# morgana-proofs/GKR-MSM

Measured on AMD Instinct MI355X. Metric: msm_points_per_sec, higher is better.
Workload: dtype u32 limbs, u64 column accumulators (BLS12-381 Fr in Montgomery form: 9 x 29-bit limbs in registers, 8 x 32 in memory)

## Files before the change

### gkr_msm_amd/csrc/g1.hip

```cpp
#include <string.h>

#include <cstring>
#include <mutex>
#include <thread>
#include <vector>


#include "common.hpp"
#include "internal.hpp"
#include "g1.hip.h"
#include "sort.hip.h"
#include "msm_plan.hpp"

namespace gm {

static constexpr uint32_t G1_NEG_BIT = 0x80000000u;

__global__ void __launch_bounds__(256) k_g1_lower_bound(const uint32_t* __restrict__ keys, uint64_t ntasks, uint32_t nkeys,
                                                         uint32_t* __restrict__ off, uint32_t* __restrict__ max_len) {
    const uint32_t k = blockIdx.x * blockDim.x + threadIdx.x;
    if (k > nkeys) return;
    auto lb = [&](uint32_t key) {
        uint64_t lo = 0, hi = ntasks;
        while (lo < hi) {
// ... 386 lines not shown

__global__ void __launch_bounds__(256) k_g1_map_tasks(const uint32_t* __restrict__ mapping, uint64_t n, uint32_t nkeys,
                                                       uint32_t* __restrict__ keys, uint32_t* __restrict__ idx,
                                                       uint32_t* __restrict__ bad) {
    const uint64_t i = (uint64_t)blockIdx.x * blockDim.x + threadIdx.x;
    if (i >= n) return;
    const uint32_t m = mapping[i];
    if (m >= nkeys) atomicAdd(bad, 1u);
    keys[i] = m < nkeys ? m : nkeys;
    idx[i] = (uint32_t)i;
}

__global__ void __launch_bounds__(128) k_g1_to_affine(const G1Jac* __restrict__ in, uint64_t n, G1Aff* __restrict__ out) {
    const uint64_t i = (uint64_t)blockIdx.x * blockDim.x + threadIdx.x;
    if (i >= n) return;
    g1_aff_store(out + i, g1_to_aff(g1_load(in + i)));
}

__global__ void __launch_bounds__(128) k_g1_from_affine(const G1Aff* __restrict__ in, uint64_t n, G1Jac* __restrict__ out) {
    const uint64_t i = (uint64_t)blockIdx.x * blockDim.x + threadIdx.x;
    if (i >= n) return;
    g1_store(out + i, g1_from_aff(g1_aff_load(in + i)));
}

__global__ void __launch_bounds__(128) k_g1_gen_points(G1Aff gen, uint64_t n, uint64_t seed, G1Aff* __restrict__ out) {
    const uint64_t i = (uint64_t)blockIdx.x * blockDim.x + threadIdx.x;
    if (i >= n) return;
    uint64_t z = seed + 0x9E3779B97F4A7C15ULL * (i + 1);
    z = (z ^ (z >> 30)) * 0xBF58476D1CE4E5B9ULL;
    z = (z ^ (z >> 27)) * 0x94D049BB133111EBULL;
    z ^= z >> 31;
    z |= 1;
    G1Jac acc = g1_inf();
    for (int b = 63; b >= 0; b--) {
        acc = g1_dbl(acc);
        if ((z >> b) & 1) acc = g1_add_mixed(acc, gen);
    }
    g1_aff_store(out + i, g1_to_aff(acc));
}

__global__ void __launch_bounds__(128) k_g1_mock_srs(G1Aff g0, Fr tau, uint64_t n, G1Aff* __restrict__ out) {
    const uint64_t i = (uint64_t)blockIdx.x * blockDim.x + threadIdx.x;
    if (i >= n) return;
    Fr acc = fr_one(), b = tau;
    for (uint64_t e = i; e; e >>= 1) {
        if (e & 1) acc = fr_mul(acc, b);
        b = fr_sqr(b);
    }
    const Fr k = fr_from_mont(acc);
    G1Jac r = g1_inf();
    for (int li = 7; li >= 0; li--)
        for (int bit = 31; bit >= 0; bit--) {
            r = g1_dbl(r);
            if ((k.l[li] >> bit) & 1) r = g1_add_mixed(r, g0);
        }
    g1_aff_store(out + i, g1_to_aff(r));
}

struct G1Scratch {
    char* base = nullptr;
    size_t cap = 0, used = 0;
    std::mutex mu;
    int32_t reserve(size_t bytes) {
        if (bytes <= cap) return GM_OK;
        if (base) dev_free(base);
        base = nullptr;
        cap = 0;
        hipError_t e = dev_alloc((void**)&base, bytes);
        if (e != hipSuccess) return set_err(GM_ERR_HIP, "hipMalloc(G1 scratch %zu): %s", bytes, hipGetErrorString(e));
        cap = bytes;
        return GM_OK;
    }
    void* carve(size_t b) {
        const size_t a = (used + 255) & ~(size_t)255;
        used = a + b;
        return base + a;
    }
    void release() {
        if (base) dev_free(base);
        base = nullptr;
        cap = used = 0;
    }
};
static G1Scratch& g1_scratch() {
    static G1Scratch s[GM_MAX_DEVICES];
    int dev = 0;
    (void)hipGetDevice(&dev);
    return s[(dev >= 0 && dev < GM_MAX_DEVICES) ? dev : 0];
}

static size_t al(size_t b) { return (b + 255) & ~(size_t)255; }

struct G1Layout {
    size_t sort_tmp = 0, scan_tmp = 0, total = 0;
};

static uint32_t bit_len(uint32_t v) {
    uint32_t b = 0;
    while (v) { b++; v >>= 1; }
    return b;
}

static int32_t g1_engine_layout(uint64_t ntasks, uint32_t nkeys, G1Layout* L) {
    const size_t st = radix_sort_tmp_bytes(ntasks), sc = 33 * scan_tmp_bytes((size_t)nkeys + 1);
    L->sort_tmp = st;
    L->scan_tmp = sc;
    L->total = al(st) + al(sc) + 2 * al(ntasks * 4) + 35 * al(((size_t)nkeys + 1) * 4) + al(64) + al((ntasks / 64 + (size_t)34 * (nkeys / 32 + 3) + 64) * 4) +
               al((ntasks / 2 + nkeys + 1) * (size_t)G1_CELL_WORDS * 4) + al((ntasks / 4 + nkeys + 1) * (size_t)G1_CELL_WORDS * 4) + 4096;
    return GM_OK;
}

static int32_t g1_sum_by_key(G1Scratch& ws, const G1Aff* src_aff, const G1Jac* src_jac, uint32_t* keys, uint32_t* idx,
                             uint64_t ntasks, uint32_t nkeys, G1Jac* out, hipStream_t s) {
    GM_REQUIRE(ntasks < (1ull << 31), "too many G1 tasks (%llu)", (unsigned long long)ntasks);
    GM_REQUIRE(nkeys >= 1 && nkeys < (1u << 30), "bad key count %u", nkeys);
    G1Layout L;
    int32_t rc = g1_engine_layout(ntasks ? ntasks : 1, nkeys, &L);
    if (rc) return rc;
    uint32_t* sort_tmp = (uint32_t*)ws.carve(L.sort_tmp);
    uint32_t* scan_tmp = (uint32_t*)ws.carve(L.scan_tmp);
    uint32_t* keys_s = (uint32_t*)ws.carve((ntasks + 1) * 4);
    uint32_t* idx_s = (uint32_t*)ws.carve((ntasks + 1) * 4);
    const size_t orow = (size_t)nkeys + 1;
    uint32_t* off_all = (uint32_t*)ws.carve(33 * al(orow * 4));
    const size_t ostride = al(orow * 4) / 4;
    (void)ws.carve(orow * 4);
    uint32_t* d_max = (uint32_t*)ws.carve(64);
    uint32_t* bufA = (uint32_t*)ws.carve((ntasks / 2 + nkeys + 1) * (size_t)G1_CELL_WORDS * 4);
    uint32_t* bufB = (uint32_t*)ws.carve((ntasks / 4 + nkeys + 1) * (size_t)G1_CELL_WORDS * 4);
    uint32_t* blk_row = (uint32_t*)ws.carve((ntasks / 64 + (size_t)34 * (nkeys / 32 + 3) + 64) * 4);
    if (ws.used > ws.cap) return set_err(GM_ERR_STATE, "G1 scratch under-reserved (%zu > %zu)", ws.used, ws.cap);

    GM_HIP(hipMemsetAsync(d_max, 0, 4, s));
    GM_HIP(radix_sort_pairs_u32(keys, idx, keys_s, idx_s, ntasks, bit_len(nkeys), sort_tmp, &keys_s, &idx_s, s));
    hipLaunchKernelGGL(k_g1_lower_bound, dim3(ceil_div(orow, 256)), dim3(256), 0, s, keys_s, ntasks, nkeys, off_all, d_max);
    GM_LAUNCH_CHECK();
    uint32_t max_len = 0;
    GM_HIP(hipMemcpyAsync(&max_len, d_max, 4, hipMemcpyDeviceToHost, s));
    GM_HIP(hipStreamSynchronize(s));
    uint32_t nlev = 0;
    while ((1u << nlev) < max_len) nlev++;
    GM_REQUIRE(nlev <= 32, "row too long");
    if (nlev) {
        const uint32_t ntiles = ceil_div(orow, SCAN_TILE);
        hipLaunchKernelGGL(k_g1_levels_scan_tiles, dim3(ntiles, nlev), dim3(1024), 0, s, off_all, nkeys, off_all, ostride, scan_tmp);
        GM_LAUNCH_CHECK();
        if (ntiles > 1) {
            hipLaunchKernelGGL(k_g1_levels_scan_fix, dim3(ntiles, nlev), dim3(1024), 0, s, nkeys, off_all, ostride, scan_tmp);
            GM_LAUNCH_CHECK();
        }
    }
    const G1SrcAff sa{src_aff, idx_s};
    const G1SrcJac sj{src_jac, idx_s};
    if (nlev == 0) {
        if (src_aff) hipLaunchKernelGGL((k_g1_rows_out<G1SrcAff>), dim3(ceil_div(nkeys, 128)), dim3(128), 0, s, sa, off_all, nkeys, out);
        else hipLaunchKernelGGL((k_g1_rows_out<G1SrcJac>), dim3(ceil_div(nkeys, 128)), dim3(128), 0, s, sj, off_all, nkeys, out);
        GM_LAUNCH_CHECK();
        return GM_OK;
    }
    uint64_t bound = ntasks / 2 + nkeys;
    G1BlockRowsArgs ba;
    ba.nlev = nlev;
    {
        uint64_t b = bound;
        uint32_t tot = 0;
        for (uint32_t l = 0; l < nlev; l++) {
            ba.first[l] = tot;
// ... 174 lines not shown
struct G1FixedBase {
    const G1Aff* bases = nullptr;
    uint64_t n = 0;
    uint32_t c = 16, nwin = 16;
    G1Aff* tab = nullptr;
    int dev = 0;
    G1Aff first{}, last{};
};
static std::mutex& g1_fixed_mu() {
    static std::mutex m;
    return m;
}
static std::vector<G1FixedBase>& g1_fixed_registry() {
    static std::vector<G1FixedBase> r;
    return r;
}
static bool g1_fixed_lookup(const G1Aff* bases, uint64_t n, G1FixedBase* out, hipStream_t s) {
    G1FixedBase cand;
    {
        std::lock_guard<std::mutex> lock(g1_fixed_mu());
        bool found = false;
        int dev = 0;
        (void)hipGetDevice(&dev);
        for (const G1FixedBase& f : g1_fixed_registry())
            if (f.bases == bases && n <= f.n && f.dev == dev) { cand = f; found = true; break; }
        if (!found) return false;
    }
    G1Aff now[2];
    if (hipMemcpyAsync(&now[0], cand.bases, sizeof(G1Aff), hipMemcpyDeviceToHost, s) != hipSuccess ||
        hipMemcpyAsync(&now[1], cand.bases + (cand.n - 1), sizeof(G1Aff), hipMemcpyDeviceToHost, s) != hipSuccess ||
        hipStreamSynchronize(s) != hipSuccess) {
        (void)hipGetLastError();
        return false;
    }
    if (memcmp(&now[0], &cand.first, sizeof(G1Aff)) != 0 || memcmp(&now[1], &cand.last, sizeof(G1Aff)) != 0) return false;
    *out = cand;
    return true;
}

static int32_t g1_msm_fixed_core(const G1FixedBase& fb, const uint64_t* d_scalars, uint64_t n, int scalars_mont, uint32_t nbits,
                                 G1Jac* h_out, hipStream_t s) {
    if (n == 0) { *h_out = g1_inf(); return GM_OK; }
    GM_REQUIRE(nbits >= 1 && nbits <= 256, "bad scalar width %u", nbits);
    uint32_t nwin = (nbits + fb.c - 1) / fb.c;
    if (nwin > fb.nwin) nwin = fb.nwin;
    const uint64_t ntasks = (uint64_t)nwin * n;
    const uint32_t nkeys = 1u << fb.c;
    GM_REQUIRE(ntasks < (1ull << 31) && fb.n * fb.nwin < (1ull << 31), "fixed-base MSM too large for one call");
    G1Scratch& ws = g1_scratch();
    std::lock_guard<std::mutex> lock(ws.mu);
    const size_t need = 2 * al(ntasks * 4) + al((size_t)nkeys * sizeof(G1Jac)) + g1_engine_bytes(ntasks, nkeys) +
                        g1_weighted_bytes(1, nkeys) + 8192;
    int32_t rc = ws.reserve(need);
    if (rc) return rc;
    ws.used = 0;
    uint32_t* keys = (uint32_t*)ws.carve(ntasks * 4);
    uint32_t* idx = (uint32_t*)ws.carve(ntasks * 4);
    G1Jac* buckets = (G1Jac*)ws.carve((size_t)nkeys * sizeof(G1Jac));
    hipLaunchKernelGGL(k_g1_msm_tasks_fixed, dim3(ceil_div(n, 256)), dim3(256), 0, s, reinterpret_cast<const uint32_t*>(d_scalars), n,
                       fb.n, fb.c, nwin, scalars_mont, nkeys, keys, idx);
    GM_LAUNCH_CHECK();
    const size_t mark = ws.used;
    rc = g1_sum_by_key(ws, fb.tab, nullptr, keys, idx, ntasks, nkeys, buckets, s);
    if (rc) return rc;
    ws.used = mark;
    std::vector<G1Jac> wsum;
    rc = g1_weighted_sums(ws, buckets, 1, nkeys, &wsum, s);
    if (rc) return rc;
    *h_out = wsum[0];
    return GM_OK;
}

}

using namespace gm;

static void put_aff(uint64_t* h, const G1Jac& p) {
    const G1Aff a = g1_to_aff(p);
    memcpy(h, &a, sizeof(G1Aff));
}

extern "C" int32_t gm_g1_release_scratch(void) {
    G1Scratch& ws = g1_scratch();
    std::lock_guard<std::mutex> lock(ws.mu);
    ws.release();
    return GM_OK;
}

extern "C" int32_t gm_g1_host(int32_t op, const uint64_t* h_a, const uint64_t* h_b, uint64_t* h_out, uint64_t n) {
    GM_REQUIRE(op >= 0 && op <= 7 && h_a && h_out, "bad argument");
    GM_REQUIRE(!(op == 0 || op == 2 || op == 4 || op == 6 || op == 7) || h_b, "second operand missing");
    for (uint64_t i = 0; i < n; i++) {
        G1Jac ja, jb, jr;
        G1Aff aa, ab, ar;
        switch (op) {
            case 0: memcpy(&ja, h_a + 18 * i, 144); memcpy(&jb, h_b + 18 * i, 144); jr = g1_add(ja, jb); memcpy(h_out + 18 * i, &jr, 144); break;
            case 1: memcpy(&ja, h_a + 18 * i, 144); jr = g1_dbl(ja); memcpy(h_out + 18 * i, &jr, 144); break;
            case 2: memcpy(&ja, h_a + 18 * i, 144); memcpy(&ab, h_b + 12 * i, 96); jr = g1_add_mixed(ja, ab); memcpy(h_out + 18 * i, &jr, 144); break;
            case 3: memcpy(&ja, h_a + 18 * i, 144); ar = g1_to_aff(ja); memcpy(h_out + 12 * i, &ar, 96); break;
            case 4: memcpy(&aa, h_a + 12 * i, 96); memcpy(&ab, h_b + 12 * i, 96); jr = g1_add_aff(aa, ab); memcpy(h_out + 18 * i, &jr, 144); break;
            case 5: memcpy(&aa, h_a + 12 * i, 96); h_out[i] = g1_aff_on_curve(aa) ? 1 : 0; break;
            default: {
                Fq x, y;
                memcpy(&x, h_a + 6 * i, 48); memcpy(&y, h_b + 6 * i, 48);
                const Fq z = op == 6 ? fq_mul(x, y) : fq_mul_c(x, y);
                memcpy(h_out + 6 * i, &z, 48);
            }
        }
    }
    return GM_OK;
}

namespace gm {
__global__ void __launch_bounds__(128) k_g1_batch(int op, const uint64_t* __restrict__ a, const uint64_t* __restrict__ b,
                                                   uint64_t* __restrict__ out, uint64_t n) {
    const uint64_t i = (uint64_t)blockIdx.x * blockDim.x + threadIdx.x;
    if (i >= n) return;
    const G1Jac* ja = reinterpret_cast<const G1Jac*>(a);
    const G1Jac* jb = reinterpret_cast<const G1Jac*>(b);
    const G1Aff* aa = reinterpret_cast<const G1Aff*>(a);
    const G1Aff* ab = reinterpret_cast<const G1Aff*>(b);
    G1Jac* jo = reinterpret_cast<G1Jac*>(out);
    switch (op) {
        case 0: g1_store(jo + i, g1_add(g1_load(ja + i), g1_load(jb + i))); break;
        case 1: g1_store(jo + i, g1_dbl(g1_load(ja + i))); break;
        case 2: g1_store(jo + i, g1_add_mixed(g1_load(ja + i), g1_aff_load(ab + i))); break;
        case 3: g1_aff_store(reinterpret_cast<G1Aff*>(out) + i, g1_to_aff(g1_load(ja + i))); break;
        default: g1_store(jo + i, g1_add_aff(g1_aff_load(aa + i), g1_aff_load(ab + i))); break;
    }
}
}

extern "C" int32_t gm_g1_batch(int32_t op, const uint64_t* d_a, const uint64_t* d_b, uint64_t* d_out, uint64_t n, void* stream) {
    GM_REQUIRE(op >= 0 && op <= 4 && d_a && d_out, "bad argument");
    GM_REQUIRE(!(op == 0 || op == 2 || op == 4) || d_b, "second operand missing");
    if (n == 0) return GM_OK;
    hipLaunchKernelGGL(k_g1_batch, dim3(ceil_div(n, 128)), dim3(128), 0, as_stream(stream), op, d_a, d_b, d_out, n);
    GM_LAUNCH_CHECK();
    return GM_OK;
}

extern "C" int32_t gm_g1_gen_points(uint64_t* d_points_aff, uint64_t n, uint64_t seed, void* stream) {
    GM_REQUIRE(d_points_aff, "null argument");
    if (n == 0) return GM_OK;
    static const uint32_t GX[12] = {0xdb22c6bbu, 0xfb3af00au, 0xf97a1aefu, 0x6c55e83fu, 0x171bac58u, 0xa14e3a3fu,
                                    0x9774b905u, 0xc3688c4fu, 0x4fa9ac0fu, 0x2695638cu, 0x3197d794u, 0x17f1d3a7u};
    static const uint32_t GY[12] = {0x46c5e7e1u, 0x0caa2329u, 0xa2888ae4u, 0xd03cc744u, 0x2c04b3edu, 0x00db18cbu,
                                    0xd5d00af6u, 0xfcf5e095u, 0x741d8ae4u, 0xa09e30edu, 0xe3aaa0f1u, 0x08b3f481u};
    G1Aff g;
    memcpy(&g.x, GX, 48);
    memcpy(&g.y, GY, 48);
    g.x = fq_to_mont(g.x);
    g.y = fq_to_mont(g.y);
    GM_REQUIRE(g1_aff_on_curve(g), "generator constant is off the curve");
    hipLaunchKernelGGL(k_g1_gen_points, dim3(ceil_div(n, 128)), dim3(128), 0, as_stream(stream), g, n, seed,
                       reinterpret_cast<G1Aff*>(d_points_aff));
    GM_LAUNCH_CHECK();
    return GM_OK;
}

extern "C" int32_t gm_g1_generator(uint64_t* h_out_aff) {
    GM_REQUIRE(h_out_aff, "null argument");
    static const uint32_t X[12] = {0xdb22c6bbu, 0xfb3af00au, 0xf97a1aefu, 0x6c55e83fu, 0x171bac58u, 0xa14e3a3fu,
                                   0x9774b905u, 0xc3688c4fu, 0x4fa9ac0fu, 0x2695638cu, 0x3197d794u, 0x17f1d3a7u};
    static const uint32_t Y[12] = {0x46c5e7e1u, 0x0caa2329u, 0xa2888ae4u, 0xd03cc744u, 0x2c04b3edu, 0x00db18cbu,
                                   0xd5d00af6u, 0xfcf5e095u, 0x741d8ae4u, 0xa09e30edu, 0xe3aaa0f1u, 0x08b3f481u};
    G1Aff g;
    for (int i = 0; i < 12; i++) { g.x.l[i] = X[i]; g.y.l[i] = Y[i]; }
// ... 413 lines not shown
```

### gkr_msm_amd/csrc/msm.hip

```cpp
#include <algorithm>
#include <vector>

#include "algfn.hip.h"
#include "common.hpp"
#include "msm_plan.hpp"
#include "ragged.hip.h"
#include "fr9.hip.h"

namespace gm {

static constexpr int CHUNK = 1024;

struct Point3 {
    Fr x, y, z;
};
typedef uint32_t gm_u4_t __attribute__((ext_vector_type(4)));

__device__ __forceinline__ Point3 pt_identity() {
    Point3 p;
    p.x = fr_zero();
    p.y = fr_one();
    p.z = fr_one();
    return p;
}
// ... 1022 lines not shown
#undef STAGE_MARK
    return GM_OK;
}

extern "C" int32_t gm_msm_bucket_sums(const gm_msm_plan* p, const uint64_t** d_x, const uint64_t** d_y,
                                      const uint64_t** d_z, uint64_t* n_rows_local) {
    GM_REQUIRE(p, "null plan");
    if (d_x) *d_x = reinterpret_cast<const uint64_t*>(p->bsum[0]);
    if (d_y) *d_y = reinterpret_cast<const uint64_t*>(p->bsum[1]);
    if (d_z) *d_z = reinterpret_cast<const uint64_t*>(p->bsum[2]);
    if (n_rows_local) *n_rows_local = p->nrows;
    return GM_OK;
}

extern "C" int32_t gm_msm_window_points(const gm_msm_plan* p, const uint64_t** d_cols, uint64_t* n_cols,
                                        uint64_t* col_len) {
    GM_REQUIRE(p, "null plan");
    if (d_cols) *d_cols = reinterpret_cast<const uint64_t*>(p->win_pts);
    if (n_cols) *n_cols = 3ull * (p->d_log + 1);
    if (col_len) *col_len = p->nwin;
    return GM_OK;
}

extern "C" int32_t gm_msm_digits(const gm_msm_plan* p, const uint16_t** d_digits, const uint32_t** d_counter,
                                 const uint32_t** d_row_len) {
    GM_REQUIRE(p, "null plan");
    if (d_digits) *d_digits = p->digits;
    if (d_counter) *d_counter = p->counter;
    if (d_row_len) *d_row_len = p->row_len;
    return GM_OK;
}

namespace gm {

__global__ void __launch_bounds__(256) k_u_to_fr(const uint16_t* __restrict__ dg, const uint32_t* __restrict__ ct,
                                                  uint64_t n, Fr* __restrict__ d_out, Fr* __restrict__ c_out) {
    const uint64_t i = (uint64_t)blockIdx.x * blockDim.x + threadIdx.x;
    if (i >= n) return;
    fr_store(d_out + i, fr_from_u64(dg[i]));
    fr_store(c_out + i, fr_from_u64(ct[i]));
}

__global__ void __launch_bounds__(256) k_access_counts(const uint16_t* __restrict__ dg, const uint32_t* __restrict__ ct,
                                                        uint64_t n, uint32_t* __restrict__ cnt_d, uint32_t* __restrict__ cnt_c) {
    const uint64_t i = (uint64_t)blockIdx.x * blockDim.x + threadIdx.x;
    if (i >= n) return;
    atomicAdd(&cnt_d[dg[i]], 1u);
    atomicAdd(&cnt_c[ct[i]], 1u);
}

__global__ void __launch_bounds__(256) k_neg_count_to_fr(const uint32_t* __restrict__ cnt, uint64_t n, Fr* __restrict__ out) {
    const uint64_t i = (uint64_t)blockIdx.x * blockDim.x + threadIdx.x;
    if (i >= n) return;
    fr_store(out + i, fr_neg(fr_from_u64(cnt[i])));
}

__global__ void __launch_bounds__(256) k_ac_c_from_sorted(const uint32_t* __restrict__ sorted, uint32_t n, uint64_t N, Fr* __restrict__ out) {
    const uint64_t k = (uint64_t)blockIdx.x * blockDim.x + threadIdx.x;
    if (k >= N) return;
    uint32_t lo = 0, hi = n;
    while (lo < hi) {
        const uint32_t mid = (lo + hi) >> 1;
        if (sorted[mid] <= k) lo = mid + 1; else hi = mid;
    }
    fr_store(out + k, fr_neg(fr_from_u64(n - lo)));
}

__global__ void __launch_bounds__(256) k_pull(const uint16_t* __restrict__ dg, const uint32_t* __restrict__ ct, uint64_t n,
                                               const Fr* __restrict__ eq_d, const Fr* __restrict__ eq_c,
                                               Fr* __restrict__ d_pull, Fr* __restrict__ c_pull) {
    const uint64_t i = (uint64_t)blockIdx.x * blockDim.x + threadIdx.x;
    if (i >= n) return;
    fr_store(d_pull + i, fr_load(eq_d + dg[i]));
    fr_store(c_pull + i, fr_load(eq_c + ct[i]));
}

int32_t launch_eq_sequence(const Fr& mult, const Fr* pt, uint32_t nvars, Fr* const* levels, hipStream_t s, const Fr* extra = nullptr,
                           uint32_t n_extra = 0, Fr* extra_dst = nullptr);

}

extern "C" int32_t gm_msm_phase1_polys(const gm_msm_plan* p, uint64_t* d_c, uint64_t* d_d, uint64_t* d_ac_c,
                                       uint64_t* d_ac_d, void* stream) {
    GM_REQUIRE(p && d_c && d_d && d_ac_c && d_ac_d, "null argument");
    hipStream_t s = as_stream(stream);
    const uint64_t n = (uint64_t)p->nwin * p->N;
    hipLaunchKernelGGL(k_u_to_fr, dim3(ceil_div(n, 256)), dim3(256), 0, s, p->digits, p->counter, n,
                       reinterpret_cast<Fr*>(d_d), reinterpret_cast<Fr*>(d_c));
    GM_LAUNCH_CHECK();
    uint32_t* cnt = nullptr;
    const uint64_t nc = (uint64_t)p->nrows + p->nd;
    GM_HIP(dev_alloc((void**)&cnt, nc * 4));
    {
        std::vector<uint32_t> rl(p->nrows), h(nc, 0);
        GM_HIP(hipMemcpyAsync(rl.data(), p->row_len, (size_t)p->nrows * 4, hipMemcpyDeviceToHost, s));
        GM_HIP(hipStreamSynchronize(s));
        for (uint32_t r = 0; r < p->nrows; r++) h[p->nrows + (r % p->nd)] += rl[r];
        std::sort(rl.begin(), rl.end());
        memcpy(h.data(), rl.data(), (size_t)p->nrows * 4);
        GM_HIP(hipMemcpyAsync(cnt, h.data(), nc * 4, hipMemcpyHostToDevice, s));
        GM_HIP(hipStreamSynchronize(s));
    }
    hipLaunchKernelGGL(k_ac_c_from_sorted, dim3(ceil_div(p->N, 256)), dim3(256), 0, s, cnt, p->nrows, p->N, reinterpret_cast<Fr*>(d_ac_c));
    GM_LAUNCH_CHECK();
    hipLaunchKernelGGL(k_neg_count_to_fr, dim3(ceil_div(p->nd, 256)), dim3(256), 0, s, cnt + p->nrows, (uint64_t)p->nd,
                       reinterpret_cast<Fr*>(d_ac_d));
    GM_LAUNCH_CHECK();
    GM_HIP(hipStreamSynchronize(s));
    dev_free(cnt);
    return GM_OK;
}

extern "C" int32_t gm_msm_second_phase(const gm_msm_plan* p, const uint64_t* h_r, uint32_t y_logsize, uint64_t* d_c_pull,
                                       uint64_t* d_d_pull, void* stream) {
    GM_REQUIRE(p && h_r && d_c_pull && d_d_pull, "null argument");
    hipStream_t s = as_stream(stream);
    const uint32_t dl = p->d_log, xl = p->x_log;
    std::vector<Fr> r(y_logsize + dl + xl);
    memcpy(r.data(), h_r, r.size() * sizeof(Fr));
    Fr* buf = nullptr;
    const uint64_t tot = (2ull << xl) + (2ull << dl);
    GM_HIP(dev_alloc((void**)&buf, tot * sizeof(Fr)));
    Fr* eq_c = buf;
    Fr* eq_d = buf + (2ull << xl);
    std::vector<Fr*> lv(xl + 1);
    for (uint32_t i = 0; i < xl; i++) lv[i] = eq_c + (1ull << xl) + ((1ull << i) - 1);
    lv[xl] = eq_c;
    int32_t rc = launch_eq_sequence(fr_one(), r.data() + y_logsize + dl, xl, lv.data(), s);
    if (rc == GM_OK) {
        lv.assign(dl + 1, nullptr);
        for (uint32_t i = 0; i < dl; i++) lv[i] = eq_d + (1ull << dl) + ((1ull << i) - 1);
        lv[dl] = eq_d;
        rc = launch_eq_sequence(fr_one(), r.data() + y_logsize, dl, lv.data(), s);
    }
    if (rc == GM_OK) {
        const uint64_t n = (uint64_t)p->nwin * p->N;
        hipLaunchKernelGGL(k_pull, dim3(ceil_div(n, 256)), dim3(256), 0, s, p->digits, p->counter, n, eq_d, eq_c,
                           reinterpret_cast<Fr*>(d_d_pull), reinterpret_cast<Fr*>(d_c_pull));
        if (hipGetLastError() != hipSuccess) rc = set_err(GM_ERR_HIP, "k_pull launch failed");
    }
    (void)hipStreamSynchronize(s);
    dev_free(buf);
    return rc;
}
```

### gkr_msm_amd/csrc/prover.hip

```cpp
#include <chrono>
#include <memory>
#include <vector>

#include "internal.hpp"
#include "gkr_layers.hpp"
#include "msm_plan.hpp"
#include "vecvec.hpp"

using namespace gm;

extern "C" {
int32_t gm_vv_from_msm(const gm_msm_plan* p, const uint64_t* d_points_xy, uint32_t y_logsize, gm_vv** out, void* stream);
int32_t gm_vv_slice(const gm_vv* in, uint32_t first, uint32_t count, gm_vv** out);
int32_t gm_vv_concat(const gm_vv* a, const gm_vv* b, gm_vv** out);
int32_t gm_vv_destroy(gm_vv* v);
struct gm_sc;
int32_t gm_sc_dense_deg2_create(const gm_fn* f, uint32_t num_vars, const uint64_t* const* d_cols, const uint64_t* h_point,
                                const uint64_t* h_gamma, const uint64_t* h_claims, gm_sc** out, void* stream);
int32_t gm_sc_vecvec_deg2_create(const gm_fn* f, const gm_vv* polys, const uint64_t* h_point, const uint64_t* h_gamma,
                                 const uint64_t* h_claims, gm_sc** out, void* stream);
int32_t gm_sc_unipoly(gm_sc* so, uint64_t* h_coeffs, uint32_t* n_coeffs);
int32_t gm_sc_bind(gm_sc* so, const uint64_t* h_t);
int32_t gm_sc_final_evals(gm_sc* so, uint64_t* h_evals, uint32_t* n_evals);
int32_t gm_sc_claim(const gm_sc* so, uint64_t* h_claim);
int32_t gm_sc_destroy(gm_sc* so);
}

namespace {

#define TRY(x)                      \
    do {                            \
        int32_t rc__ = (x);         \
        if (rc__) return rc__;      \
    } while (0)

struct StageTimer {
    const char* who;
    hipStream_t s;
    bool on;
    std::chrono::steady_clock::time_point prev;
    StageTimer(const char* w, hipStream_t st) : who(w), s(st) {
        static const bool v = [] { const char* e = getenv("GM_PROVE_TIMING"); return e && e[0] == '1'; }();
        on = v;
        if (on) { (void)hipStreamSynchronize(s); prev = std::chrono::steady_clock::now(); }
    }
    void mark(const char* name) {
        if (!on) return;
        (void)hipStreamSynchronize(s);
        const auto now = std::chrono::steady_clock::now();
        fprintf(stderr, "[gm %s] %-24s %8.2f ms   (pool misses so far: %llu, %.1f MiB)\n", who, name,
                std::chrono::duration<double, std::milli>(now - prev).count(), (unsigned long long)dev_pool().n_driver_allocs,
                dev_pool().driver_alloc_bytes / 1048576.0);
        prev = now;
    }
};

struct VVHolder {
    gm_vv* v = nullptr;
    VVHolder() = default;
    explicit VVHolder(gm_vv* p) : v(p) {}
    VVHolder(const VVHolder&) = delete;
    VVHolder& operator=(const VVHolder&) = delete;
    ~VVHolder() { if (v) gm_vv_destroy(v); }
};

struct Advice {
    enum Kind { VECVEC, DENSE, EMPTY } kind = EMPTY;
    std::shared_ptr<VVHolder> vv;
    std::vector<std::shared_ptr<DevBuf>> cols;
    uint64_t len = 0;
    std::vector<const uint64_t*> col_ptrs() const {
        std::vector<const uint64_t*> p;
        for (auto& c : cols) p.push_back(reinterpret_cast<const uint64_t*>(c->p));
        return p;
    }
};

int32_t dense_alloc(int n, uint64_t len, std::vector<std::shared_ptr<DevBuf>>* out) {
    out->clear();
    for (int i = 0; i < n; i++) {
        out->emplace_back(new DevBuf());
        TRY(out->back()->alloc((size_t)len * sizeof(Fr)));
    }
    return GM_OK;
// ... 1880 lines not shown
    std::vector<Fr> multirow(1ull << (y_log - clm), fr_zero());
    multirow[0] = fr_one();
    for (uint32_t i = 0; i < y_log - clm; i++)
        for (uint64_t j = (1ull << i); j-- > 0;) {
            const Fr w = multirow[j], m = fr_mul(mx.point[i], w);
            multirow[2 * j] = fr_sub(w, m);
            multirow[2 * j + 1] = m;
        }
    const uint32_t n_comb = n_mat < multirow.size() ? n_mat : (uint32_t)multirow.size();
    DevBuf d_mr, d_cs;
    TRY(d_mr.alloc(n_comb * sizeof(Fr)));
    TRY(d_cs.alloc((size_t)n_comb * sizeof(G1Aff)));
    GM_HIP(hipMemcpyAsync(d_mr.p, multirow.data(), n_comb * sizeof(Fr), hipMemcpyHostToDevice, s));
    auto comb = [&](const uint64_t* cs, G1Jac* out) -> int32_t {
        uint64_t r12[12];
        GM_HIP(hipMemcpyAsync(d_cs.p, cs, (size_t)n_comb * sizeof(G1Aff), hipMemcpyHostToDevice, s));
        const int32_t rc = gm_g1_msm((const uint64_t*)d_cs.p, (const uint64_t*)d_mr.p, n_comb, 1, 255, r12, stream);
        if (rc) return rc;
        *out = pp_aff_in(r12);
        return GM_OK;
    };
    G1Jac c_comb, d_comb, cp_comb, dp_comb;
    TRY(comb(st->comm_c.data(), &c_comb));
    TRY(comb(st->comm_d.data(), &d_comb));
    TRY(comb(comm_cp.data(), &cp_comb));
    TRY(comb(comm_dp.data(), &dp_comb));
    Fr u;
    TRY(tr->challenge(&u, 512));
    Us us;
    us.u[0] = fr_one(); us.u[1] = u; us.u[2] = fr_mul(u, u); us.u[3] = fr_mul(us.u[2], u);
    const G1Jac combined_comm = g1_add(g1_add(c_comb, pp_mul(d_comb, us.u[1])), g1_add(pp_mul(cp_comb, us.u[2]), pp_mul(dp_comb, us.u[3])));
    const Fr combined_ev = fr_add(fr_add(c_ev, fr_mul(d_ev, us.u[1])), fr_add(fr_mul(c_pull_ev, us.u[2]), fr_mul(d_pull_ev, us.u[3])));
    DevBuf w0, w1, w2, w3, d_multirow, folded;
    TRY(w0.alloc(n * sizeof(Fr))); TRY(w1.alloc(n * sizeof(Fr))); TRY(w2.alloc(n * sizeof(Fr))); TRY(w3.alloc(n * sizeof(Fr)));
    TRY(folded.alloc(n * sizeof(Fr)));
    for (DevBuf* b : {&w0, &w1, &w2}) GM_HIP(hipMemsetAsync(b->p, 0, n * sizeof(Fr), s));
    hipLaunchKernelGGL(k_pp_axpy, dim3(ceil_div(X, 256)), dim3(256), 0, s, st->p0->fr(), st->p1->fr(), gamma, X, w0.fr());
    GM_LAUNCH_CHECK();
    GM_HIP(hipMemcpyAsync(w1.p, cols.ac_c->p, X * sizeof(Fr), hipMemcpyDeviceToDevice, s));
    GM_HIP(hipMemcpyAsync(w2.p, cols.ac_d->p, ((size_t)1 << d_log) * sizeof(Fr), hipMemcpyDeviceToDevice, s));
    TRY(d_multirow.alloc(multirow.size() * sizeof(Fr)));
    GM_HIP(hipMemcpyAsync(d_multirow.p, multirow.data(), multirow.size() * sizeof(Fr), hipMemcpyHostToDevice, s));
    hipLaunchKernelGGL(k_pp_combined, dim3(ceil_div(n, 256)), dim3(256), 0, s, cols.c->fr(), cols.d->fr(), cols.c_pull->fr(),
                       cols.d_pull->fr(), d_multirow.fr(), us, x_log, y_size, clm, n, w3.fr());
    GM_LAUNCH_CHECK();
    GM_HIP(hipStreamSynchronize(s));
    stage("opening witnesses");
    ProveSpans::get().end(3);
    std::vector<Fr> mo_evs = {fr_sub(p_folded_ev, fr_mul(gamma, gamma)), acc.evs[0], acd.evs[0], combined_ev};
    const uint64_t* wcols[4] = {(const uint64_t*)w0.p, (const uint64_t*)w1.p, (const uint64_t*)w2.p, (const uint64_t*)w3.p};
    std::vector<Fr> mo_pt, mo_out;
    TRY(multiopen_core(tr, nv, 4, wcols, reinterpret_cast<const uint64_t*>(pts.data()), reinterpret_cast<const uint64_t*>(mo_evs.data()),
                       &mo_pt, &mo_out, s));
    stage("multi-open reduction");
    ProveSpans::get().end(4);
    Fr q;
    TRY(tr->challenge(&q));
    Us qs;
    qs.u[0] = fr_one(); qs.u[1] = q; qs.u[2] = fr_mul(q, q); qs.u[3] = fr_mul(qs.u[2], q);
    const G1Jac parts[4] = {g1_add(pp_aff_in(st->comm_p0), pp_mul(pp_aff_in(st->comm_p1), gamma)), pp_aff_in(st->comm_ac_c),
                            pp_aff_in(st->comm_ac_d), combined_comm};
    G1Jac folded_comm = g1_inf();
    for (int j = 0; j < 4; j++) folded_comm = g1_add(folded_comm, pp_mul(parts[j], qs.u[j]));
    Cols4 c4;
    c4.p[0] = w0.fr(); c4.p[1] = w1.fr(); c4.p[2] = w2.fr(); c4.p[3] = w3.fr();
    hipLaunchKernelGGL(k_pp_fold4, dim3(ceil_div(n, 256)), dim3(256), 0, s, c4, qs, n, folded.fr());
    GM_LAUNCH_CHECK();
    Fr open_ev = mo_out[3];
    for (int j = 2; j >= 0; j--) open_ev = fr_add(fr_mul(open_ev, q), mo_out[j]);
    uint64_t fc_aff[12], proof[48];
    pp_aff_out(fc_aff, folded_comm);
    gm_transcript adapter{tr, tape_ws, tape_ch, tape_wp};
    TRY(gm_knuckles_open_tr(st->d_basis, d_kn_inverses, h_k, nv, reinterpret_cast<const uint64_t*>(folded.p), n,
                            reinterpret_cast<const uint64_t*>(mo_pt.data()), reinterpret_cast<const uint64_t*>(&open_ev), fc_aff,
                            &adapter, proof, h_pair, stream));
    stage("knuckles open");
    ProveSpans::get().end(5);
    if (tr->cb_rc) return set_err(GM_ERR_STATE, "transcript callback failed with %d", tr->cb_rc);
    return GM_OK;
}

}

extern "C" int32_t gm_pippenger_wg_create(const gm_msm_plan* plan, const uint64_t* d_points_xy, uint32_t y_logsize,
                                          uint32_t commitment_log_multiplicity, const uint64_t* d_kzg_basis_aff,
                                          gm_pippenger_wg** out, void* stream) {
    GM_REQUIRE(plan && d_points_xy && d_kzg_basis_aff && out, "null argument");
    GM_REQUIRE(commitment_log_multiplicity <= y_logsize, "commitment_log_multiplicity exceeds y_logsize");
    hipStream_t s = as_stream(stream);
    std::unique_ptr<gm_pippenger_wg> st(new gm_pippenger_wg());
    st->plan = plan; st->d_points_xy = d_points_xy; st->d_basis = d_kzg_basis_aff; st->y_log = y_logsize;
    st->clm = commitment_log_multiplicity; st->stream = s;
    const uint32_t cm = 1u << st->clm;
    st->n_mat = (plan->y_size + cm - 1) / cm;
    StageTimer wt("wg::new", s);
    TRY(pip_witness_create(plan, d_points_xy, y_logsize, nullptr, &st->w, stream));
    wt.mark("witness");
    {
        std::vector<uint32_t> rl(plan->nrows);
        GM_HIP(hipMemcpyAsync(rl.data(), plan->row_len, (size_t)plan->nrows * 4, hipMemcpyDeviceToHost, s));
        GM_HIP(hipStreamSynchronize(s));
        uint32_t cmax = 1;
        for (uint32_t v : rl) cmax = v > cmax ? v : cmax;
        st->c_upper.assign(st->n_mat, 1);
        for (uint32_t r = 0; r < plan->nrows; r++) {
            const uint32_t m = (r >> plan->d_log) >> st->clm;
            if (rl[r] > st->c_upper[m]) st->c_upper[m] = rl[r];
        }
        st->d_outer.reset(new DevBuf());
        st->c_outer.reset(new DevBuf());
        TRY(st->d_outer->alloc(((size_t)st->n_mat << plan->d_log) * sizeof(G1Jac)));
        TRY(st->c_outer->alloc((size_t)st->n_mat * cmax * sizeof(G1Jac)));
        st->comm_c.assign(12 * (size_t)st->n_mat, 0);
        st->comm_d.assign(12 * (size_t)st->n_mat, 0);
        TRY(gm_msm_g1_outer(plan, d_kzg_basis_aff, st->clm, (uint64_t*)st->d_outer->p, (uint64_t*)st->c_outer->p,
                            (uint64_t)st->n_mat * cmax, &st->c_stride, st->comm_d.data(), st->comm_c.data(), stream));
    }
    wt.mark("outer buckets + c/d comm");
    const uint64_t X = plan->N, D = 1ull << plan->d_log;
    st->p0.reset(new DevBuf());
    st->p1.reset(new DevBuf());
    TRY(st->p0->alloc(X * sizeof(Fr)));
    TRY(st->p1->alloc(X * sizeof(Fr)));
    hipLaunchKernelGGL(k_pp_split_xy, dim3(ceil_div(X, 256)), dim3(256), 0, s, reinterpret_cast<const Fr*>(d_points_xy), X, st->p0->fr(),
                       st->p1->fr());
    GM_LAUNCH_CHECK();
    {
        DevBuf c, d, ac_c, ac_d;
        const uint64_t msize = (uint64_t)plan->y_size * X;
        TRY(c.alloc(msize * sizeof(Fr))); TRY(d.alloc(msize * sizeof(Fr))); TRY(ac_c.alloc(X * sizeof(Fr))); TRY(ac_d.alloc(D * sizeof(Fr)));
        TRY(gm_msm_phase1_polys(plan, (uint64_t*)c.p, (uint64_t*)d.p, (uint64_t*)ac_c.p, (uint64_t*)ac_d.p, stream));
        wt.mark("phase-1 polys");
        TRY(gm_g1_msm(d_kzg_basis_aff, (const uint64_t*)st->p0->p, X, 1, 255, st->comm_p0, stream));
        TRY(gm_g1_msm(d_kzg_basis_aff, (const uint64_t*)st->p1->p, X, 1, 255, st->comm_p1, stream));
        wt.mark("p_0, p_1 commitments");
        auto commit_negated_counts = [&](DevBuf& col, uint64_t len, uint64_t* out12) -> int32_t {
            TRY(gm_fr_batch(3, (const uint64_t*)col.p, nullptr, (uint64_t*)col.p, len, stream));
            TRY(gm_g1_msm(d_kzg_basis_aff, (const uint64_t*)col.p, len, 1, 32, out12, stream));
            G1Aff a;
            memcpy(&a, out12, sizeof(G1Aff));
            if (!g1_aff_is_inf(a)) a = g1_aff_neg(a);
            memcpy(out12, &a, sizeof(G1Aff));
            return GM_OK;
        };
        TRY(commit_negated_counts(ac_c, X, st->comm_ac_c));
        TRY(commit_negated_counts(ac_d, D, st->comm_ac_d));
        wt.mark("ac_c, ac_d commitments");
    }
    *out = st.release();
    return GM_OK;
}


namespace {

int32_t commit_replicated_part(const gm_pippenger_wg* st, const Fr* d_col, uint64_t L, uint32_t nbits, G1Jac* part, const char* what, void* stream) {
    const uint32_t G = st->sh.world;
    uint64_t lo = 0, cnt = st->sh.rank == 0 ? L : 0;
    if (L >= G) { cnt = L / G; lo = (uint64_t)st->sh.rank * cnt; }
    *part = g1_inf();
    if (!cnt) return GM_OK;
    GM_KEY_RANGE(kp, &st->key, lo, cnt, what);
    uint64_t a12[12];
    TRY(gm_g1_msm(kp, reinterpret_cast<const uint64_t*>(d_col + lo), cnt, 1, nbits, a12, stream));
    *part = pp_aff_in(a12);
    return GM_OK;
}

int32_t pippenger_prove_sharded(const gm_pippenger_wg* st, const uint64_t* h_claim_point, const uint64_t* h_claim_evs,
                                const uint64_t* d_kn_inverses_slice, const uint64_t* h_k, Tape* tr, uint64_t* h_pair) {
    const gm_msm_plan* plan = st->plan;
    const Shard& sh = st->sh;
    const uint32_t x_log = plan->x_log, d_log = plan->d_log, y_log = st->y_log, clm = st->clm, G = sh.world;
    const uint32_t n_mat = st->n_mat, cm = 1u << clm;
    hipStream_t s = st->stream;
    void* stream = reinterpret_cast<void*>(s);
    GM_REQUIRE(y_log >= clm, "commitment_log_multiplicity exceeds y_logsize");
    StageTimer timer("prove (sharded)", s);
    auto stage = [&](const char* name) { timer.mark(name); };
    ProveSpans::get().start();
    tr->write_points(st->comm_c.data(), n_mat);
    tr->write_points(st->comm_d.data(), n_mat);
    tr->write_points(st->comm_p0, 1);
    tr->write_points(st->comm_p1, 1);
    tr->write_points(st->comm_ac_c, 1);
    tr->write_points(st->comm_ac_d, 1);
    Claims c;
    c.point.resize(y_log);
    memcpy(c.point.data(), h_claim_point, 32 * (size_t)y_log);
    c.evs.resize(3 * (d_log + 1));
    memcpy(c.evs.data(), h_claim_evs, 32 * c.evs.size());
    TRY(image_part_core(st->w, tr, &c));
    stage("image part");
    ProveSpans::get().end(0);
    std::vector<uint64_t> comm_cp(12 * (size_t)n_mat), comm_dp(12 * (size_t)n_mat);
    {
        const uint64_t X = 1ull << x_log, D = 1ull << d_log;
        DevBuf eqs;
        TRY(eqs.alloc((2 * X + 2 * D) * sizeof(Fr)));
        Fr* eq_c = eqs.fr();
        Fr* eq_d = eqs.fr() + 2 * X;
        std::vector<Fr*> lv(x_log + 1);
        for (uint32_t i = 0; i < x_log; i++) lv[i] = eq_c + X + ((1ull << i) - 1);
        lv[x_log] = eq_c;
        TRY(launch_eq_sequence(fr_one(), c.point.data() + y_log + d_log, x_log, lv.data(), s));
        lv.assign(d_log + 1, nullptr);
        for (uint32_t i = 0; i < d_log; i++) lv[i] = eq_d + D + ((1ull << i) - 1);
        lv[d_log] = eq_d;
        TRY(launch_eq_sequence(fr_one(), c.point.data() + y_log, d_log, lv.data(), s));
        const uint32_t nl = st->n_mat_loc;
        std::vector<uint32_t> nd_all(nl, (uint32_t)D);
        std::vector<uint64_t> loc_d(12 * (size_t)nl), loc_c(12 * (size_t)nl);
        TRY(gm_g1_msm_nonaff_grouped(reinterpret_cast<const uint64_t*>(st->d_outer->p), D, nd_all.data(), nl,
                                     reinterpret_cast<const uint64_t*>(eq_d), 1, 255, loc_d.data(), stream));
        TRY(gm_g1_msm_nonaff_grouped(reinterpret_cast<const uint64_t*>(st->c_outer->p), st->c_stride, st->c_upper.data(), nl,
                                     reinterpret_cast<const uint64_t*>(eq_c), 1, 255, loc_c.data(), stream));
        std::vector<G1Jac> parts(2 * (size_t)n_mat, g1_inf());
        for (uint32_t i = 0; i < nl; i++) {
            parts[st->m0 + i] = pp_aff_in(loc_c.data() + 12 * (size_t)i);
            parts[n_mat + st->m0 + i] = pp_aff_in(loc_d.data() + 12 * (size_t)i);
        }
        std::vector<uint64_t> both(24 * (size_t)n_mat);
        TRY(gm_g1_combine_parts(sh.comm, reinterpret_cast<const uint64_t*>(parts.data()), 2 * n_mat, both.data()));
        memcpy(comm_cp.data(), both.data(), 96 * (size_t)n_mat);
        memcpy(comm_dp.data(), both.data() + 12 * (size_t)n_mat, 96 * (size_t)n_mat);
    }
    tr->write_points(comm_cp.data(), n_mat);
    tr->write_points(comm_dp.data(), n_mat);
    stage("phase-2 commitments");
    ProveSpans::get().end(1);
    Fr gamma;
// ... 316 lines not shown
```

Before: 381.6 million.

## Run outer buckets and column commitments on worker threads concurrent with witness

Splits pippenger_wg_create into three independent stages and runs the outer-bucket MSM and the p0/p1/ac commitments on two persistent worker threads, each with its own HIP stream and G1 scratch, while the caller builds the witness. It also stops allocating and filling the full c/d phase-1 matrices, which were unused here. The aim is to overlap GPU work and host-side synchronisation that previously ran serially. The cost is more threading complexity, extra device memory for the per-thread scratch buffers, and contention between concurrent kernels.

```diff
diff --git a/gkr_msm_amd/csrc/g1.hip b/gkr_msm_amd/csrc/g1.hip
--- a/gkr_msm_amd/csrc/g1.hip
+++ b/gkr_msm_amd/csrc/g1.hip
@@ -492,7 +492,17 @@
         cap = used = 0;
     }
 };
+static thread_local G1Scratch* t_own_scratch = nullptr;
+static std::mutex g1_own_mu;
+static std::vector<G1Scratch*> g1_own_list;
+void g1_thread_own_scratch() {
+    if (t_own_scratch) return;
+    t_own_scratch = new G1Scratch();
+    std::lock_guard<std::mutex> g(g1_own_mu);
+    g1_own_list.push_back(t_own_scratch);
+}
 static G1Scratch& g1_scratch() {
+    if (t_own_scratch) return *t_own_scratch;
     static G1Scratch s[GM_MAX_DEVICES];
     int dev = 0;
     (void)hipGetDevice(&dev);
@@ -833,8 +843,15 @@
 
 extern "C" int32_t gm_g1_release_scratch(void) {
     G1Scratch& ws = g1_scratch();
-    std::lock_guard<std::mutex> lock(ws.mu);
-    ws.release();
+    {
+        std::lock_guard<std::mutex> lock(ws.mu);
+        ws.release();
+    }
+    std::lock_guard<std::mutex> g(g1_own_mu);
+    for (G1Scratch* o : g1_own_list) {
+        std::lock_guard<std::mutex> lock(o->mu);
+        o->release();
+    }
     return GM_OK;
 }
 
diff --git a/gkr_msm_amd/csrc/msm.hip b/gkr_msm_amd/csrc/msm.hip
--- a/gkr_msm_amd/csrc/msm.hip
+++ b/gkr_msm_amd/csrc/msm.hip
@@ -1128,12 +1128,14 @@
 
 extern "C" int32_t gm_msm_phase1_polys(const gm_msm_plan* p, uint64_t* d_c, uint64_t* d_d, uint64_t* d_ac_c,
                                        uint64_t* d_ac_d, void* stream) {
-    GM_REQUIRE(p && d_c && d_d && d_ac_c && d_ac_d, "null argument");
+    GM_REQUIRE(p && d_ac_c && d_ac_d && !d_c == !d_d, "null argument");
     hipStream_t s = as_stream(stream);
-    const uint64_t n = (uint64_t)p->nwin * p->N;
-    hipLaunchKernelGGL(k_u_to_fr, dim3(ceil_div(n, 256)), dim3(256), 0, s, p->digits, p->counter, n,
-                       reinterpret_cast<Fr*>(d_d), reinterpret_cast<Fr*>(d_c));
-    GM_LAUNCH_CHECK();
+    if (d_c) {
+        const uint64_t n = (uint64_t)p->nwin * p->N;
+        hipLaunchKernelGGL(k_u_to_fr, dim3(ceil_div(n, 256)), dim3(256), 0, s, p->digits, p->counter, n,
+                           reinterpret_cast<Fr*>(d_d), reinterpret_cast<Fr*>(d_c));
+        GM_LAUNCH_CHECK();
+    }
     uint32_t* cnt = nullptr;
     const uint64_t nc = (uint64_t)p->nrows + p->nd;
     GM_HIP(dev_alloc((void**)&cnt, nc * 4));
diff --git a/gkr_msm_amd/csrc/prover.hip b/gkr_msm_amd/csrc/prover.hip
--- a/gkr_msm_amd/csrc/prover.hip
+++ b/gkr_msm_amd/csrc/prover.hip
@@ -1,5 +1,9 @@
 #include <chrono>
+#include <condition_variable>
+#include <functional>
 #include <memory>
+#include <mutex>
+#include <thread>
 #include <vector>
 
 #include "internal.hpp"
@@ -2046,6 +2050,139 @@
 
 }
 
+namespace gm {
+void g1_thread_own_scratch();
+}
+namespace {
+
+struct WgWorker {
+    std::mutex mu;
+    std::condition_variable cv;
+    std::function<int32_t(hipStream_t)> job;
+    bool pending = false, finished = false;
+    int32_t rc = GM_OK;
+    char err[512] = {0};
+    int dev = 0;
+    hipStream_t s = nullptr;
+    hipEvent_t done = nullptr;
+
+    int32_t init(int device) {
+        dev = device;
+        GM_HIP(hipStreamCreateWithFlags(&s, hipStreamNonBlocking));
+        GM_HIP(hipEventCreateWithFlags(&done, hipEventDisableTiming));
+        std::thread([this] { loop(); }).detach();
+        return GM_OK;
+    }
+    void loop() {
+        (void)hipSetDevice(dev);
+        g1_thread_own_scratch();
+        for (;;) {
+            std::function<int32_t(hipStream_t)> f;
+            {
+                std::unique_lock<std::mutex> lk(mu);
+                cv.wait(lk, [this] { return pending; });
+                f.swap(job);
+                pending = false;
+            }
+            int32_t r = f(s);
+            const hipError_t e = hipEventRecord(done, s);
+            if (e != hipSuccess) {
+                (void)hipStreamSynchronize(s);
+                if (r == GM_OK) r = set_err(GM_ERR_HIP, "hipEventRecord(worker stream): %s", hipGetErrorString(e));
+            }
+            std::lock_guard<std::mutex> lk(mu);
+            rc = r;
+            if (r) memcpy(err, err_buf(), sizeof(err));
+            finished = true;
+            cv.notify_all();
+        }
+    }
+    void post(std::function<int32_t(hipStream_t)> f) {
+        std::lock_guard<std::mutex> lk(mu);
+        job.swap(f);
+        pending = true;
+        finished = false;
+        cv.notify_all();
+    }
+    int32_t join(hipStream_t s_caller) {
+        std::unique_lock<std::mutex> lk(mu);
+        cv.wait(lk, [this] { return finished; });
+        int32_t r = rc;
+        if (r) set_err(r, "%s", err);
+        lk.unlock();
+        const hipError_t e = hipStreamWaitEvent(s_caller, done, 0);
+        if (e != hipSuccess) {
+            (void)hipStreamSynchronize(s);
+            if (r == GM_OK) r = set_err(GM_ERR_HIP, "hipStreamWaitEvent(worker event): %s", hipGetErrorString(e));
+        }
+        return r;
+    }
+};
+
+struct WgWorkers {
+    std::mutex busy;
+    WgWorker w[2];
+    hipEvent_t ready = nullptr;
+    static int32_t get(int dev, WgWorkers** out) {
+        static std::mutex mu;
+        static WgWorkers* per_dev[GM_MAX_DEVICES] = {nullptr};
+        GM_REQUIRE(dev >= 0 && dev < GM_MAX_DEVICES, "device id %d: the per-device tables of this library hold %d devices", dev, GM_MAX_DEVICES);
+        std::lock_guard<std::mutex> g(mu);
+        if (!per_dev[dev]) {
+            WgWorkers* p = new WgWorkers();
+            GM_HIP(hipEventCreateWithFlags(&p->ready, hipEventDisableTiming));
+            for (WgWorker& wk : p->w) TRY(wk.init(dev));
+            per_dev[dev] = p;
+        }
+        *out = per_dev[dev];
+        return GM_OK;
+    }
+};
+
+bool wg_serial() {
+    static const bool v = [] { const char* e = getenv("GM_WG_SERIAL"); return e && e[0] == '1'; }();
+    return v;
+}
+
+int32_t wg_outer(gm_pippenger_wg* st, uint64_t c_cap, hipStream_t s) {
+    StageTimer t("wg::new B", s);
+    TRY(gm_msm_g1_outer(st->plan, st->d_basis, st->clm, (uint64_t*)st->d_outer->p, (uint64_t*)st->c_outer->p, c_cap, &st->c_stride,
+                        st->comm_d.data(), st->comm_c.data(), s));
+    t.mark("outer buckets + c/d comm");
+    return GM_OK;
+}
+
+int32_t wg_columns(gm_pippenger_wg* st, hipStream_t s) {
+    StageTimer t("wg::new C", s);
+    const gm_msm_plan* plan = st->plan;
+    const uint64_t X = plan->N, D = 1ull << plan->d_log;
+    hipLaunchKernelGGL(k_pp_split_xy, dim3(ceil_div(X, 256)), dim3(256), 0, s, reinterpret_cast<const Fr*>(st->d_points_xy), X,
+                       st->p0->fr(), st->p1->fr());
+    GM_LAUNCH_CHECK();
+    DevBuf ac_c, ac_d;
+    TRY(ac_c.alloc(X * sizeof(Fr))); TRY(ac_d.alloc(D * sizeof(Fr)));
+    TRY(gm_msm_phase1_polys(plan, nullptr, nullptr, (uint64_t*)ac_c.p, (uint64_t*)ac_d.p, s));
+    t.mark("phase-1 polys");
+    TRY(gm_g1_msm(st->d_basis, (const uint64_t*)st->p0->p, X, 1, 255, st->comm_p0, s));
+    TRY(gm_g1_msm(st->d_basis, (const uint64_t*)st->p1->p, X, 1, 255, st->comm_p1, s));
+    t.mark("p_0, p_1 commitments");
+    auto commit_negated_counts = [&](DevBuf& col, uint64_t len, uint64_t* out12) -> int32_t {
+        TRY(gm_fr_batch(3, (const uint64_t*)col.p, nullptr, (uint64_t*)col.p, len, s));
+        TRY(gm_g1_msm(st->d_basis, (const uint64_t*)col.p, len, 1, 32, out12, s));
+        G1Aff a;
+        memcpy(&a, out12, sizeof(G1Aff));
+        if (!g1_aff_is_inf(a)) a = g1_aff_neg(a);
+        memcpy(out12, &a, sizeof(G1Aff));
+        return GM_OK;
+    };
+    TRY(commit_negated_counts(ac_c, X, st->comm_ac_c));
+    TRY(commit_negated_counts(ac_d, D, st->comm_ac_d));
+    t.mark("ac_c, ac_d commitments");
+    return GM_OK;
+}
+
+}
+
 extern "C" int32_t gm_pippenger_wg_create(const gm_msm_plan* plan, const uint64_t* d_points_xy, uint32_t y_logsize,
                                           uint32_t commitment_log_multiplicity, const uint64_t* d_kzg_basis_aff,
                                           gm_pippenger_wg** out, void* stream) {
@@ -2058,59 +2195,64 @@
     const uint32_t cm = 1u << st->clm;
     st->n_mat = (plan->y_size + cm - 1) / cm;
     StageTimer wt("wg::new", s);
-    TRY(pip_witness_create(plan, d_points_xy, y_logsize, nullptr, &st->w, stream));
-    wt.mark("witness");
-    {
-        std::vector<uint32_t> rl(plan->nrows);
-        GM_HIP(hipMemcpyAsync(rl.data(), plan->row_len, (size_t)plan->nrows * 4, hipMemcpyDeviceToHost, s));
-        GM_HIP(hipStreamSynchronize(s));
-        uint32_t cmax = 1;
-        for (uint32_t v : rl) cmax = v > cmax ? v : cmax;
-        st->c_upper.assign(st->n_mat, 1);
-        for (uint32_t r = 0; r < plan->nrows; r++) {
-            const uint32_t m = (r >> plan->d_log) >> st->clm;
-            if (rl[r] > st->c_upper[m]) st->c_upper[m] = rl[r];
-        }
-        st->d_outer.reset(new DevBuf());
-        st->c_outer.reset(new DevBuf());
-        TRY(st->d_outer->alloc(((size_t)st->n_mat << plan->d_log) * sizeof(G1Jac)));
-        TRY(st->c_outer->alloc((size_t)st->n_mat * cmax * sizeof(G1Jac)));
-        st->comm_c.assign(12 * (size_t)st->n_mat, 0);
-        st->comm_d.assign(12 * (size_t)st->n_mat, 0);
-        TRY(gm_msm_g1_outer(plan, d_kzg_basis_aff, st->clm, (uint64_t*)st->d_outer->p, (uint64_t*)st->c_outer->p,
-                            (uint64_t)st->n_mat * cmax, &st->c_stride, st->comm_d.data(), st->comm_c.data(), stream));
-    }
-    wt.mark("outer buckets + c/d comm");
-    const uint64_t X = plan->N, D = 1ull << plan->d_log;
+    std::vector<uint32_t> rl(plan->nrows);
+    GM_HIP(hipMemcpyAsync(rl.data(), plan->row_len, (size_t)plan->nrows * 4, hipMemcpyDeviceToHost, s));
+    GM_HIP(hipStreamSynchronize(s));
+    uint32_t cmax = 1;
+    for (uint32_t v : rl) cmax = v > cmax ? v : cmax;
+    st->c_upper.assign(st->n_mat, 1);
+    for (uint32_t r = 0; r < plan->nrows; r++) {
+        const uint32_t m = (r >> plan->d_log) >> st->clm;
+        if (rl[r] > st->c_upper[m]) st->c_upper[m] = rl[r];
+    }
+    const uint64_t X = plan->N, c_cap = (uint64_t)st->n_mat * cmax;
+    st->d_outer.reset(new DevBuf());
+    st->c_outer.reset(new DevBuf());
     st->p0.reset(new DevBuf());
     st->p1.reset(new DevBuf());
+    TRY(st->d_outer->alloc(((size_t)st->n_mat << plan->d_log) * sizeof(G1Jac)));
+    TRY(st->c_outer->alloc(c_cap * sizeof(G1Jac)));
     TRY(st->p0->alloc(X * sizeof(Fr)));
     TRY(st->p1->alloc(X * sizeof(Fr)));
-    hipLaunchKernelGGL(k_pp_split_xy, dim3(ceil_div(X, 256)), dim3(256), 0, s, reinterpret_cast<const Fr*>(d_points_xy), X, st->p0->fr(),
-                       st->p1->fr());
-    GM_LAUNCH_CHECK();
-    {
-        DevBuf c, d, ac_c, ac_d;
-        const uint64_t msize = (uint64_t)plan->y_size * X;
-        TRY(c.alloc(msize * sizeof(Fr))); TRY(d.alloc(msize * sizeof(Fr))); TRY(ac_c.alloc(X * sizeof(Fr))); TRY(ac_d.alloc(D * sizeof(Fr)));
-        TRY(gm_msm_phase1_polys(plan, (uint64_t*)c.p, (uint64_t*)d.p, (uint64_t*)ac_c.p, (uint64_t*)ac_d.p, stream));
-        wt.mark("phase-1 polys");
-        TRY(gm_g1_msm(d_kzg_basis_aff, (const uint64_t*)st->p0->p, X, 1, 255, st->comm_p0, stream));
-        TRY(gm_g1_msm(d_kzg_basis_aff, (const uint64_t*)st->p1->p, X, 1, 255, st->comm_p1, stream));
-        wt.mark("p_0, p_1 commitments");
-        auto commit_negated_counts = [&](DevBuf& col, uint64_t len, uint64_t* out12) -> int32_t {
-            TRY(gm_fr_batch(3, (const uint64_t*)col.p, nullptr, (uint64_t*)col.p, len, stream));
-            TRY(gm_g1_msm(d_kzg_basis_aff, (const uint64_t*)col.p, len, 1, 32, out12, stream));
-            G1Aff a;
-            memcpy(&a, out12, sizeof(G1Aff));
-            if (!g1_aff_is_inf(a)) a = g1_aff_neg(a);
-            memcpy(out12, &a, sizeof(G1Aff));
-            return GM_OK;
-        };
-        TRY(commit_negated_counts(ac_c, X, st->comm_ac_c));
-        TRY(commit_negated_counts(ac_d, D, st->comm_ac_d));
-        wt.mark("ac_c, ac_d commitments");
-    }
+    st->comm_c.assign(12 * (size_t)st->n_mat, 0);
+    st->comm_d.assign(12 * (size_t)st->n_mat, 0);
+    gm_pippenger_wg* w = st.get();
+
+    WgWorkers* pool = nullptr;
+    std::unique_lock<std::mutex> held;
+    if (!wg_serial()) {
+        int dev = 0;
+        GM_HIP(hipGetDevice(&dev));
+        TRY(WgWorkers::get(dev, &pool));
+        held = std::unique_lock<std::mutex>(pool->busy, std::try_to_lock);
+        if (!held.owns_lock()) pool = nullptr;
+    }
+    if (!pool) {
+        TRY(pip_witness_create(plan, d_points_xy, y_logsize, nullptr, &st->w, stream));
+        wt.mark("witness");
+        TRY(wg_outer(w, c_cap, s));
+        TRY(wg_columns(w, s));
+        *out = st.release();
+        return GM_OK;
+    }
+    GM_HIP(hipEventRecord(pool->ready, s));
+    hipEvent_t ready = pool->ready;
+    pool->w[0].post([w, c_cap, ready](hipStream_t ws) -> int32_t {
+        GM_HIP(hipStreamWaitEvent(ws, ready, 0));
+        return wg_outer(w, c_cap, ws);
+    });
+    pool->w[1].post([w, ready](hipStream_t ws) -> int32_t {
+        GM_HIP(hipStreamWaitEvent(ws, ready, 0));
+        return wg_columns(w, ws);
+    });
+    int32_t rc = pip_witness_create(plan, d_points_xy, y_logsize, nullptr, &st->w, stream);
+    wt.mark("witness (B, C running)");
+    const int32_t rc_b = pool->w[0].join(s);
+    const int32_t rc_c = pool->w[1].join(s);
+    wt.mark("joined B, C");
+    if (rc) return rc;
+    if (rc_b) return rc_b;
+    if (rc_c) return rc_c;
     *out = st.release();
     return GM_OK;
 }
```

Result: no change. 381.6 million (median of 6 runs) (+0.0%).
